# revollllt/FP8_quantization

Measured on AMD Instinct MI355X. Metric: ImageNet val images/sec, ResNet-18 FP8 approx_v9, higher is better.
Workload: dtype fp32; 1 GPU; resnet18 E4M3 approx_v9 forward (dnsmp_factor=3, withComp=False, with_s2nn2s_opt, quant_btw_mult_accu, res_quantizer, fixed ranges), ImageNet-shaped synthetic batch, random-init weights with BN statistics estimated on 4 synthetic batches; global_batch=1024, per_gpu_batch=1024, approx_macs_per_image=1814073344, parallelism=dp1

## Files before the change

### fp8_quantization_amd/csrc/fp8approx.hip

```cpp
#include <hip/hip_runtime.h>
#include <stdint.h>
#include <string.h>

#include <algorithm>
#include <atomic>
#include <cmath>
#include <cstdlib>
#include <cstdio>
#include <map>
#include <mutex>
#include <string>
#include <vector>

#include "../../include/fp8approx.h"
#include "fp8approx_common.h"
#include "fp8approx_launch.h"
#include "gemm_f8mx.h"
#include "gemm_v5mx.h"
#include "gemm_tt.h"
#include "gemm_tt16.h"
#include "gemm_dense.h"
#include "conv_tbx.h"
#include "gemm_check.h"
#include "fq_mse.h"
// ... 439 lines not shown
        const float *s = ap_sm + t * ps;
        float acc = 0.0f;
        for (int r = 0; r < kh; ++r)
            for (int c = 0; c < kw; ++c) acc += s[r * W + c];
        y[P0 + t] = acc / (float)(kh * kw);
    }
}

__global__ __launch_bounds__(256) void max_pool2d_s2k3_kernel(const float *x, float *y, int64_t planes, int H, int W,
                                                             int Ho) {
    const int Wq = W / 8;
    const int64_t total = planes * Ho * Wq;
    for (int64_t idx = (int64_t)blockIdx.x * blockDim.x + threadIdx.x; idx < total;
         idx += (int64_t)gridDim.x * blockDim.x) {
        const int q = (int)(idx % Wq);
        const int64_t t = idx / Wq;
        const int ho = (int)(t % Ho);
        const int64_t pl = t / Ho;
        const float *xp = x + pl * H * W;
        float m[4] = {-INFINITY, -INFINITY, -INFINITY, -INFINITY};
        const int c0 = 8 * q;
#pragma unroll
        for (int ky = 0; ky < 3; ++ky) {
            const int hi = 2 * ho - 1 + ky;
            if ((unsigned)hi >= (unsigned)H) continue;
            const float *r = xp + (int64_t)hi * W + c0;
            const float4 a = *reinterpret_cast<const float4 *>(r), b = *reinterpret_cast<const float4 *>(r + 4);
            const float v[9] = {c0 > 0 ? r[-1] : -INFINITY, a.x, a.y, a.z, a.w, b.x, b.y, b.z, b.w};
#pragma unroll
            for (int o = 0; o < 4; ++o)
#pragma unroll
                for (int kx = 0; kx < 3; ++kx) {
                    if (o == 0 && kx == 0 && c0 == 0) continue;
                    const float u = v[2 * o + kx];
                    m[o] = (u > m[o] || u != u) ? u : m[o];
                }
        }
        *reinterpret_cast<float4 *>(y + (pl * Ho + ho) * (int64_t)(W / 2) + 4 * q) = make_float4(m[0], m[1], m[2], m[3]);
    }
}

static void launch_f8mx(const GemmArgs &a, hipStream_t s) {
    if (a.Mw == 2) {
        launch_f8mx_xf1(a, s);
        launch_f8mx_xf2(a, s);
    } else {
        launch_f8mx_xf0(a, s);
    }
}

static int g_opt_xm_ncg = getenv("FP8A_XM_NCG") ? atoi(getenv("FP8A_XM_NCG")) : 0;
static int g_opt_xm_sign_rows = getenv("FP8A_XM_SIGN_ROWS") ? atoi(getenv("FP8A_XM_SIGN_ROWS")) : 1;
static int g_opt_xm_pipe = getenv("FP8A_XM_PIPE") ? atoi(getenv("FP8A_XM_PIPE")) != 0 : 1;
static int g_opt_fq_fast = getenv("FP8A_FQ_FAST") ? atoi(getenv("FP8A_FQ_FAST")) != 0 : 1;
static int xm_ncg(int64_t N) {
    const int forced = g_opt_xm_ncg;
    if (forced == 1 || forced == 2 || forced == 4) return forced;
    int best = 4;
    int64_t bp = (N + 63) / 64 * 64;
    for (int c : {2, 1}) {
        const int64_t pad = (N + 16 * c - 1) / (16 * c) * (16 * c);
        if (pad < bp) {
            bp = pad;
            best = c;
        }
    }
    return best;
}

static void launch_fast(int mode, const GemmArgs &a, hipStream_t s) {
    const int64_t tiles = ((a.M + BM - 1) / BM) * ((a.N + BN - 1) / BN);
    const dim3 grid((unsigned)(tiles * a.splits));
    if (mode == TM_V5) {
        if (a.aw && a.wfmt == 4) launch_v5mx(a, s);
        else launch_fast_p0(TM_V5, false, a, grid, s);
        return;
    }
    if (mode == TM_QAMAA) {
        launch_fast_p0(TM_QAMAA, false, a, grid, s);
        return;
    }
    if (a.aw && (a.wfmt == 1 || a.wfmt == 2)) {
        launch_tt(a, grid, s);
        return;
    }
    if (mode == TM_F8) {
        if (a.aw || a.af32) launch_f8mx(a, s);
        else launch_fast_p3(TM_F8, false, a, grid, s);
        return;
    }
    const bool s2n = a.flags & F_S2N, q = a.flags & F_QBMA, gc = a.flags & F_GCLIP;
    if (s2n) q ? launch_fast_p3(mode, gc, a, grid, s) : launch_fast_p2(mode, gc, a, grid, s);
    else q ? launch_fast_p1(mode, gc, a, grid, s) : launch_fast_p0(mode, gc, a, grid, s);
}

static int check_format(int E, int Mw) {
    if (E < 1 || Mw < 1 || Mw > 5 || E > 6 || E + Mw > 8)
        return fail(FP8A_EFORMAT, "Invalid combination of expo_width and mant_width");
    return FP8A_OK;
}

constexpr size_t FLAG_BYTES = 256;

enum { PATH_F8MX = 0, PATH_TT = 1, PATH_TT16 = 2, PATH_FAST = 3, PATH_EXACT = 4, PATH_DENSE = 5, PATH_V5MX = 6,
       PATH_N = 7 };
static std::atomic<uint64_t> g_paths[PATH_N];
// ... 311 lines not shown
        ++g_paths[PATH_EXACT];
        gemm_exact_kernel<<<eblocks, 256, 0, s>>>(a);
        return hip_check("fp8a exact gemm launch");
    }
    if (ws == nullptr || ws_bytes < FLAG_BYTES) return fail(FP8A_EINVAL, "matmul workspace too small");
    static const bool no_units = getenv("FP8A_NO_UNITS") != nullptr;
    const size_t head = ws_bytes >= head_bytes(a.M, a.N) ? head_bytes(a.M, a.N) : FLAG_BYTES;
    ArenaLease lease;
    const int cap = stream_capturing(s);
    if (cap < 0) return hip_check("fp8a stream capture query");
    if (cap ? !capture_lease(s, ws, ws_bytes, head, lease) : !flag_arena(s, head_bytes(a.M, a.N), lease))
        return lease_error();
    a.flag = lease.mine;
    a.flag_out = (uint32_t *)ws;
    a.arena_clr = lease.clr;
    a.arena_clr16 = lease.clr16;
    a.nur = (a.M + 63) / 64;
    a.nuc = (a.N + 63) / 64;
    a.urow = no_units || (cap && head < head_bytes(a.M, a.N)) ? nullptr : (uint8_t *)a.flag + FLAG_BYTES;
    a.ucol = no_units ? nullptr : a.urow + a.nur;
    a.utile = no_units ? nullptr : a.ucol + a.nuc;
    a.splits = choose_splits(a.M, a.N, a.K);
    if (a.splits > 1 && ws_bytes < head + splitk_bytes(a.M, a.N, a.K)) a.splits = 1;
    const int64_t kt = (a.K + BK - 1) / BK;
    a.kchunk = ((kt + a.splits - 1) / a.splits) * BK;
    a.part = a.splits > 1 ? (float *)((char *)ws + head) : nullptr;
    a.aw = nullptr;
    const bool tt = mode != TM_F8 && tt_form(a.Mw, a.flags, a.tab);
    const bool v5mx = v5mx_form(a.Mw, a.flags, mode);
    if ((mode == TM_F8 || tt || v5mx) && !no_mx()) {
        const int64_t kpad = kt * BK, npad = (a.N + BN - 1) / BN * BN;
        const size_t off = head + (a.splits > 1 ? splitk_bytes(a.M, a.N, a.K) : 0);
        const int64_t a_words = xm_a_words(a);
        const WordImage wi = word_image(a.H, a.W, a.ph, a.pw);
        a.awH = wi.H; a.awW = wi.W; a.awph = wi.ph; a.awpw = wi.pw;
        const bool fits32 = a_words < (1ll << 30) && kpad * npad * 4 < (1ll << 32);
        if (fits32 && ws_bytes >= off + xm_operand_bytes(a.N, a.K, a_words)) {
            char *base = (char *)ws + off;
            a.aw = (const uint32_t *)base;
            a.awld = kpad;
            a.bqw = (const uint2 *)(base + align256((size_t)a_words * 4));
            a.lutw = (const uint32_t *)(base + align256((size_t)a_words * 4) + xm_b_bytes(kpad, npad));
            a.ebr = (const uint16_t *)((const char *)a.lutw + 16384);
            a.xm_vmin = 0;
            if (mode == TM_F8) (void)xm_table_form(a.tab, a.Mw, &a.xm_vmin);
            a.npad = npad;
            a.ttf7 = 0;
            for (int i = 0; tt && i < (1 << (2 * a.Mw)); ++i) a.ttf7 |= a.tab.raw[i] < 0;
            a.wfmt = v5mx ? 4 : tt ? (tt16_form(a.Mw, a.ttf7, a.K) ? 2 : 1) : 0;
            if (a.wfmt == 1 && !g_opt_tt_band) a.ebr = nullptr;
            a.xncg = tt ? 4 : xm_ncg(a.N);
            a.xm_signs = g_opt_xm_sign_rows;
            a.xm_pipe = g_opt_xm_pipe;
            a.skcnt = nullptr;
            if (a.splits > 1 && g_opt_splitk_fixup && a.wfmt == 0 && a.Mw == 3) {
                a.skcnt = (uint32_t *)((char *)ws + head + splitk_part_bytes(a.splits, a.M, a.N));
                a.sk_words = splitk_counter_words(a.M, a.N);
            }
            const bool use_img = a.in_img != nullptr && !tt && a.conv && a.fqin.mx != nullptr;
            if (use_img) a.aw = a.in_img + 64;
            a.af32 = !tt && !v5mx && !use_img && xm_af32(a) ? 1 : 0;
            const int64_t rows = a.conv ? a.M / (a.Ho * a.Wo) : a.M, cols = a_words / std::max<int64_t>(rows, 1);
            dim3 ga((unsigned)std::min<int64_t>((cols + 255) / 256, 64), (unsigned)std::min<int64_t>(rows, 1024));
            {
                const int64_t hw = a.H * a.W, lim0 = a.conv ? cols : a.K, istride = a.conv ? a.Cin * hw : a.lda;
                const float *in0 = a.conv ? a.X + a.cbase * hw : a.A;
                const bool flat = !(a.conv && (a.awph | a.awpw)) && lim0 % 4 == 0 && cols % 4 == 0 && istride % 4 == 0 &&
                                  ((uintptr_t)in0 & 15) == 0 && ((uintptr_t)a.aw & 15) == 0;
                if (flat) ga = dim3((unsigned)std::max<int64_t>(1, std::min<int64_t>((a_words / 4 + 1023) / 1024, 8192)), 1);
            }
            if (use_img) {
                a.gate = a.in_img;
                xm_decode_a<<<ga.y == 1 ? dim3(std::min(ga.x, 512u)) : dim3(std::min(ga.x, 8u), std::min(ga.y, 64u)), 256, 0,
                              s>>>(a);
                a.gate = nullptr;
            } else if (!a.af32) {
                xm_decode_a<<<ga, 256, 0, s>>>(a);
            }
            if (v5mx) {
                const unsigned gb = (unsigned)std::min<int64_t>((kpad * npad + 255) / 256, 4096);
                v5mx_decode_b<<<gb, 256, 0, s>>>(a, kpad);
            } else if (tt) {
                const unsigned gb = (unsigned)std::min<int64_t>((kpad * npad + 255) / 256, 4096);
                tt_decode_b<<<gb, 256, 0, s>>>(a, kpad);
            } else {
                const unsigned gb = (unsigned)std::min<int64_t>((kpad * npad / 2 + 255) / 256, 4096);
                xm_decode_b<<<gb, 256, 0, s>>>(a, kpad);
            }
            rc = hip_check("fp8a operand pre-decode launch");
            if (rc) return rc;
        }
    }
    if (a.fqin.mx && !a.aw)
        return fail(FP8A_EINVAL, "internal: fused input quantization without the matrix-core path");
    if (mode == TM_F8 && a.Mw != 3 && !a.aw) mode = mode0;
    ++g_paths[!a.aw ? PATH_FAST : a.wfmt == 0 ? PATH_F8MX : a.wfmt == 1 ? PATH_TT : a.wfmt == 4 ? PATH_V5MX : PATH_TT16];
    if (a.em.w != nullptr && (a.em.form == 2 || (a.aw && a.wfmt != 0 && a.splits == 1) || a.post_act == 2)) {
        if (dev_fill(a.em.invalid, 1, sizeof(uint32_t), s) != hipSuccess) return hip_check("fp8a word image header");
        a.em.w = nullptr;
    }
    KernelEv kev{};
    if (g_ktime && !cap) {
        kev.a = pool_event();
        kev.b = pool_event();
        kev.path = !a.aw ? PATH_FAST : a.wfmt == 0 ? PATH_F8MX : a.wfmt == 1 ? PATH_TT : a.wfmt == 4 ? PATH_V5MX : PATH_TT16;
        kev.dispatches = (a.aw && ((a.wfmt == 0 && a.Mw == 2) || a.wfmt == 2)) ? 2 : 1;
// ... 264 lines not shown
size_t fp8a_flag_arena_slot_bytes(fp8a_stream_t stream) {
    int dev = 0;
    if (hipGetDevice(&dev) != hipSuccess) return 0;
    std::lock_guard<std::mutex> lock(g_arena_mu);
    const auto it = g_arenas.find({dev, (uintptr_t)stream});
    return it == g_arenas.end() ? 0 : it->second.slot;
}

int fp8a_kernel_timing(int enable) {
    const int old = g_ktime ? 1 : 0;
    g_ktime = enable != 0;
    return old;
}

int fp8a_kernel_time(double *out, int reset) {
    if (out == nullptr) return fail(FP8A_EINVAL, "null pointer");
    for (int i = 0; i < 4 * PATH_N; ++i) out[i] = 0.0;
    for (const KernelEv &e : g_kev) {
        if (hipEventSynchronize(e.b) != hipSuccess) return hip_check("fp8a_kernel_time");
        float ms = 0.0f;
        if (hipEventElapsedTime(&ms, e.a, e.b) != hipSuccess) return hip_check("fp8a_kernel_time");
        out[4 * e.path] += ms;
        out[4 * e.path + 1] += 1.0;
        out[4 * e.path + 2] += e.dispatches;
        out[4 * e.path + 3] += e.macs;
    }
    if (reset) {
        for (const KernelEv &e : g_kev) {
            g_evpool.push_back(e.a);
            g_evpool.push_back(e.b);
        }
        g_kev.clear();
    }
    return FP8A_OK;
}

static int g_opt_mse_group = getenv("FP8A_MSE_GROUP") ? atoi(getenv("FP8A_MSE_GROUP")) != 0 : 1;

int fp8a_set_option(const char *name, int value) {
    if (name == nullptr) return fail(FP8A_EINVAL, "null pointer");
    if (strcmp(name, "xm_ncg") == 0) {
        const int old = g_opt_xm_ncg;
        g_opt_xm_ncg = value;
        return old;
    }
    if (strcmp(name, "xm_sign_rows") == 0) {
        const int old = g_opt_xm_sign_rows;
        g_opt_xm_sign_rows = value != 0;
        return old;
    }
    if (strcmp(name, "xm_pipe") == 0) {
        const int old = g_opt_xm_pipe;
        g_opt_xm_pipe = value != 0;
        return old;
    }
    if (strcmp(name, "splitk_fixup") == 0) {
        const int old = g_opt_splitk_fixup;
        g_opt_splitk_fixup = value != 0;
        return old;
    }
    if (strcmp(name, "splitk") == 0) {
        const int old = g_opt_splitk;
        g_opt_splitk = std::max(0, value);
        return old;
    }
    if (strcmp(name, "fq_fast") == 0) {
        const int old = g_opt_fq_fast;
        g_opt_fq_fast = value != 0;
        return old;
    }
    if (strcmp(name, "af32_maxct") == 0) {
        const int old = g_opt_af32_maxct;
        g_opt_af32_maxct = std::max(0, value);
        return old;
    }
    if (strcmp(name, "tt_band") == 0) {
        const int old = g_opt_tt_band;
        g_opt_tt_band = value;
        return old;
    }
    if (strcmp(name, "tt16_mink") == 0) {
        const int old = g_opt_tt16_mink;
        g_opt_tt16_mink = std::max(0, value);
        return old;
    }
    if (strcmp(name, "tbx_rw") == 0) {
        const int old = g_opt_tbx_rw;
        g_opt_tbx_rw = value;
        return old;
    }
    if (strcmp(name, "tbs") == 0) {
        const int old = g_opt_tbs;
        g_opt_tbs = value;
        return old;
    }
    if (strcmp(name, "dw_lds") == 0) {
        const int old = g_opt_dw_lds;
        g_opt_dw_lds = std::min(65536, std::max(4096, value));
        return old;
    }
    if (strcmp(name, "dw_target") == 0) {
        const int old = g_opt_dw_target;
        g_opt_dw_target = std::max(256, value);
        return old;
    }
    if (strcmp(name, "dn_direct") == 0) {
// ... 1316 lines not shown
```

### fp8_quantization_amd/csrc/fp8approx_common.h

```cpp
#pragma once
#include <hip/hip_runtime.h>
#include <stdint.h>
#include <string.h>

#include <algorithm>
#include <atomic>
#include <cmath>
#include <cstdlib>
#include <cstdio>
#include <string>

#include "../../include/fp8approx.h"
#include "fp8approx_device.h"

namespace fp8a {

enum TMode : int { TM_NONE = 0, TM_W1U = 1, TM_W2S1 = 2, TM_W2U1 = 3, TM_W2S2 = 4, TM_W2U2 = 5, TM_LUT = 6,
                   TM_QAMAA = 7 ,
                   TM_V5 = 8 ,
                   TM_F8 = 9  };

struct TablePack {
    uint32_t rows[64][2];
    int8_t raw[1024];
// ... 32 lines not shown
}
__device__ __forceinline__ FqFast fq_fast_k(float mx, float bias, int M) {
    return FqFast{(uint32_t)(128 - (int)bias) << 23, ((uint32_t)(23 - M) << 23) | 0x00400000u, mx};
}
__device__ __forceinline__ float fq_apply_fast(float xc, const FqFast &k) {
    const uint32_t u = __float_as_uint(xc);
    const float C = __uint_as_float(max(u & 0x7F800000u, k.emn) + k.cadd);
    const float q = (xc + C) - C;
    return __uint_as_float((__float_as_uint(q) & 0x7FFFFFFFu) | (u & 0x80000000u));
}
template <bool FQF>
__device__ __forceinline__ float fq_apply_f(float v, float mx, float bias, int M, int sign_bits, const FqFast &k) {
    if (FQF) {
        const float xc = fminf(fmaxf(v, sign_bits ? -k.mx : 0.0f), k.mx);
        return k.emn ? fq_apply_fast(xc, k) : fq_apply_lit(xc, bias, M);
    }
    return fq_apply_lit(fminf(fmaxf(v, sign_bits ? -mx : 0.0f), mx), bias, M);
}

struct EmitW {
    uint32_t *w;
    uint32_t *invalid;
    int awH, awW, awph, awpw;
    int Wo;
    uint32_t hw_mul, hw_shift, wo_mul, wo_shift;
    uint32_t hw;
    FqIn fq;
    const int32_t *bR;
    int Mw;
    int form;
};

struct GemmArgs {
    const float *A;
    int64_t lda;
    const float *B;
    int64_t sbk, sbn;
    float *C;
    int64_t ldc;
    int64_t M, N, K;
    int E, Mw;
    uint32_t kexp, kdc;
    const int32_t *bA;
    const int32_t *bB;
    int64_t bBs;
    const int32_t *bR;
    uint32_t flags;
    int nchw;
    int64_t hw, ctot, coff;
    uint32_t *flag;
    uint8_t *urow, *ucol, *utile;
    int64_t nur, nuc;
    int splits;
    int64_t kchunk;
    float *part;
    uint32_t *skcnt;
    int64_t sk_words;
    int conv;
    const float *X;
    int64_t Cin, H, W, Ho, Wo, cbase;
    int kh, kw, sh, sw, ph, pw, dh, dw;
    uint32_t kk_mul, kk_shift, kw_mul, kw_shift;
    const float *qmax;
    int qE, qM, qsign;
    const float2 *ep;
    int ep_act;
    float ep_lo, ep_hi;
    const uint32_t *aw;
    int64_t awld, aw_c;
    int64_t awH, awW;
    int awph, awpw;
    int wfmt;
    int ttf7;
    int af32;
    int xncg;
    int xm_signs;
    int fq_fast;
    const uint2 *bqw;
    const uint32_t *lutw;
    const uint16_t *ebr;
    int xm_vmin;
    int xm_pipe;
    int64_t npad;
    FqIn fqin;
    float *fq_bias;
    int32_t *fq_ibias;
    const float *res;
    int post_act;
    float post_lo, post_hi;
    FqIn post_fq;
    EmitW em;
    const uint32_t *gate;
    const uint32_t *in_img;
    TablePack tab;
    uint32_t *flag_out;
    uint4 *arena_clr;
    uint32_t arena_clr16;
    float *post_bout;
    int32_t *post_ibout;
};

constexpr uint32_t FB_ANY = 1u, FB_ALL = 32u;
constexpr uint32_t FB_HALF = 64u;
constexpr uint8_t UT_EXACT = 1u, UT_HALF = 2u;

__device__ __forceinline__ uint32_t fb_bits(const GemmArgs &p, bool all = false) {
// ... 430 lines not shown
```

### fp8_quantization_amd/csrc/gemm_f8mx.h

```cpp
#pragma once
#include "fp8approx_common.h"

namespace fp8a {

typedef int xm_v8i __attribute__((ext_vector_type(8)));
typedef float xm_v16f __attribute__((ext_vector_type(16)));
typedef float xm_v4f __attribute__((ext_vector_type(4)));
typedef short xm_s2 __attribute__((ext_vector_type(2)));
typedef unsigned short xm_u2 __attribute__((ext_vector_type(2)));
typedef __bf16 xm_b2 __attribute__((ext_vector_type(2)));

constexpr int XM_NPAIR = 81;
constexpr int XM_LUT_WORDS = XM_NPAIR * 8;
static_assert(XM_SIGN_BIT == (8u << XM_ROW_SHIFT) && XM_ROW_MASK == (15u << XM_ROW_SHIFT), "A word row field");
constexpr int XBK = 8;
constexpr int XM_TTK = 16 * 32 + 16;
constexpr int XM_CP = BN + 1;

template <int XF>
struct XmFmt {
    static constexpr int M = XF ? 2 : 3;
    static constexpr int XB = XF ? 15 : 7;
};
__device__ __forceinline__ bool xm_needs_halving(const GemmArgs &p, bool af32, int bA, int bR) {
// ... 362 lines not shown
                if ((cb & 0x7FFFFFFFu) == 0u) continue;
                const int e = (int)((cb >> 23) & 0xFFu) - 127;
                emax = max(emax, e);
                emin = min(emin, e);
            }
            const_cast<uint16_t *>(p.ebr)[i] = (uint16_t)((emax + 128) | ((emin + 128) << 8));
            bmax = max(bmax, (uint32_t)(emax + 128));
        }
        wave_max_atomic(p.flag + 2, bmax);
    }
    if (__syncthreads_or(bad ? 1 : 0) && threadIdx.x == 0) atomicOr(p.flag, fb_bits(p, biasbad));
}
#else
__global__ void xm_decode_b(const GemmArgs p, int64_t kpad);
#endif

#if FP8A_OWN_F8MX
#ifndef FP8A_CLOCK_STAMP
#define FP8A_CLOCK_STAMP 0
#endif
__device__ unsigned long long g_clk[3];
__device__ unsigned long long g_xm_sign[2];
#if FP8A_CLOCK_STAMP
#define FP8A_CLK_BEGIN const uint64_t clk_t0 = __builtin_amdgcn_s_memtime(), clk_r0 = __builtin_amdgcn_s_memrealtime();
#define FP8A_CLK_END                                                                                   \
    if (threadIdx.x == 0) {                                                                            \
        const uint64_t clk_t1 = __builtin_amdgcn_s_memtime(), clk_r1 = __builtin_amdgcn_s_memrealtime(); \
        atomicAdd(&g_clk[0], (unsigned long long)(clk_t1 - clk_t0));                                   \
        atomicAdd(&g_clk[1], (unsigned long long)(clk_r1 - clk_r0));                                   \
        atomicAdd(&g_clk[2], 1ull);                                                                    \
    }
#else
#define FP8A_CLK_BEGIN
#define FP8A_CLK_END
#endif
#ifndef XM_WAVES
#define XM_WAVES 5
#endif
#ifndef XM_WAVES_PLAIN
#define XM_WAVES_PLAIN (XM_BDMA ? 6 : XM_WAVES)
#endif
template <bool AF32, bool EMIT> struct XmWaves { static constexpr int value = XM_WAVES; };
template <> struct XmWaves<false, false> { static constexpr int value = XM_WAVES_PLAIN; };
#ifndef XM_PIPE_EMIT64
#define XM_PIPE_EMIT64 1
#endif
template <int NCG, bool EMIT, bool FIX> struct XmPipe { static constexpr int value = 1; };
#ifndef XM_PIPE_PLAIN64
#define XM_PIPE_PLAIN64 2
#endif
template <> struct XmPipe<4, false, false> { static constexpr int value = XM_PIPE_PLAIN64; };
template <> struct XmPipe<4, true, false> { static constexpr int value = XM_PIPE_EMIT64; };
template <bool EMIT> struct XmPipe<1, EMIT, true> { static constexpr int value = 0; };
template <int NCG, int RB, bool AF32, int XF, bool EMIT, bool FIX = false, int PIPE = 0>
__global__ __launch_bounds__(256, (XmWaves<AF32, EMIT>::value)) void gemm_f8mx_kernel(const GemmArgs p) {
    static_assert(PIPE == 0 || (!AF32 && XF != 2), "PIPE: the word-staged plain forms only");
    using Cf = XmCfg<NCG, RB>;
    constexpr int XM = XmFmt<XF>::M, XB = XmFmt<XF>::XB;
    constexpr int NT = Cf::NT, BMT = Cf::BMT, BNT = Cf::BNT, TTK = Cf::TTK, APR = Cf::APR;
    constexpr int BU = Cf::BU, NBU = Cf::NBU, TXN = Cf::TXN, SR = Cf::SR, CP = Cf::CP;
    __shared__ __attribute__((aligned(16))) typename Cf::Smem smu;
    auto &sm = smu.st;
    FP8A_CLK_BEGIN

    const int tid = threadIdx.x, lane = tid & 63, wv = tid >> 6;
    const int wvu = __builtin_amdgcn_readfirstlane(wv);
    const int wc = wvu % NCG, wr = wvu / NCG;
    const int64_t num_mt = (p.M + BMT - 1) / BMT;
    const int64_t tiles = num_mt * ((p.N + BNT - 1) / BNT);
    const int64_t bid = (int64_t)blockIdx.x % tiles, split = (int64_t)blockIdx.x / tiles;
    const int64_t m0 = (bid % num_mt) * BMT;
    const int64_t n0 = (bid / num_mt) * BNT;
    bool both = true;
    if (!AF32 && p.xm_signs)
        both = __any(__hip_atomic_load(p.flag + (lane < XM_SIGN_NW ? XM_SIGN_W0 + lane : 3), __ATOMIC_RELAXED,
                                       __HIP_MEMORY_SCOPE_WORKGROUP) != 0u) != 0;
    if (XF != 2 && blockIdx.x == 0 && tid == 0) atomicAdd(&g_xm_sign[both ? 1 : 0], 1ull);
    if (XF == 2 && !xm_half_gate(p, m0, BMT, n0, BNT)) return;
    const int kbeg = (int)(split * p.kchunk), kend = (int)min(p.K, (int64_t)kbeg + p.kchunk), K32 = (int)p.K;
    const int bR = *p.bR;
    float fmx = 0.0f, fbias = 0.0f;
    int bA = 0;
    bool abad = false, biasbad = false;
    if (AF32) {
        fmx = p.fqin.mx ? *p.fqin.mx : 0.0f;
        fbias = p.fqin.mx ? fq_bias(fmx, p.fqin.E, p.fqin.M) : 0.0f;
        bA = p.fqin.mx ? (int)fbias : *p.bA;
        if (p.fqin.mx && blockIdx.x == 0 && tid == 0) {
            *p.fq_bias = fbias;
            *p.fq_ibias = bA;
        }
        biasbad = !(xm_bias_ok(bA) && xm_bias_ok(bR));
    }
    const uint32_t emnA = (uint32_t)(128 - bA) << 23;

    for (int e = 4 * tid; e < XM_LUT_WORDS; e += 4 * NT)
        *reinterpret_cast<uint4 *>(&sm.lut[e]) = *reinterpret_cast<const uint4 *>(&p.lutw[e]);

    const uint32_t hq8 = (uint32_t)(p.npad / 2) * 8u;
    const int q4 = tid & 3, btx = (tid >> 3) % TXN;
    constexpr int BKU = 2 * (NT / (8 * TXN));
    const int bkk0 = 2 * (tid / (8 * TXN)) + ((tid >> 2) & 1);
    const uint32_t boff0 = (uint32_t)(kbeg + bkk0) * hq8 + (uint32_t)(n0 / 2 + 2 * btx) * 8u;
    const bool build = NBU % NT == 0 || tid < NBU;
#if XM_BDMA
    const float *bsrc = reinterpret_cast<const float *>(p.bqw) +
                        ((size_t)(kbeg + tid / TXN) * (hq8 / 4) + (size_t)(n0 / 2 + 2 * (tid % TXN)) * 2);
    (void)boff0;
#else
// ... 125 lines not shown
        for (int i = 0; i < APR; ++i)
            *reinterpret_cast<uint2 *>(&sm.aw[akp][2 * (arow + 64 * i)]) = make_uint2(wa[i][0], wa[i][1]);
        if (build) {
            auto pk = [](uint32_t v, xm_u2 ad) { return __builtin_bit_cast(uint32_t, __builtin_bit_cast(xm_u2, v) + ad); };
            auto unit_b = [&](int u) {
#if XM_BDMA
                return sm.bw[(bkk0 + u * BKU) * TXN + btx];
#else
                return wbq[u];
#endif
            };
            if (both) {
#pragma unroll
                for (int u = 0; u < BU; ++u) {
                    const uint4 b = unit_b(u);
                    const uint2 s0 = *reinterpret_cast<const uint2 *>(lut + b.y + 8 * q4);
                    const uint2 s1 = *reinterpret_cast<const uint2 *>(lut + b.w + 8 * q4);
                    const xm_u2 a0 = __builtin_bit_cast(xm_u2, b.x), a1 = __builtin_bit_cast(xm_u2, b.z);
                    const xm_u2 n0 = __builtin_bit_cast(xm_u2, b.x ^ 0x80008000u), n1 = __builtin_bit_cast(xm_u2, b.z ^ 0x80008000u);
                    uint32_t *d = &sm.tt[bkk0 + u * BKU][btx * 32 + q4 * 4];
                    *reinterpret_cast<uint4 *>(d) = make_uint4(pk(s0.x, a0), pk(s1.x, a1), pk(s0.y, a0), pk(s1.y, a1));
                    *reinterpret_cast<uint4 *>(d + 16) = make_uint4(pk(s0.x, n0), pk(s1.x, n1), pk(s0.y, n0), pk(s1.y, n1));
                }
            } else {
#pragma unroll
                for (int u = 0; u < BU; ++u) {
                    uint4 b = unit_b(u);
                    asm volatile("" : "+v"(b.x), "+v"(b.z));
                    const uint2 s0 = *reinterpret_cast<const uint2 *>(lut + b.y + 8 * q4);
                    const uint2 s1 = *reinterpret_cast<const uint2 *>(lut + b.w + 8 * q4);
                    const xm_u2 a0 = __builtin_bit_cast(xm_u2, b.x), a1 = __builtin_bit_cast(xm_u2, b.z);
                    uint32_t *d = &sm.tt[bkk0 + u * BKU][btx * 32 + q4 * 4];
                    *reinterpret_cast<uint4 *>(d) = make_uint4(pk(s0.x, a0), pk(s1.x, a1), pk(s0.y, a0), pk(s1.y, a1));
                }
            }
        }
        __syncthreads();
        if (k0 + XBK < kend) load_tile(k0 + XBK);

        {
            const int r16 = lane & 15, g = lane >> 4;
            const uint32_t base = wvo + (uint32_t)(2 * g) * (uint32_t)(TTK * 4);
            const char *tt0 = reinterpret_cast<const char *>(&sm.tt[0][0]);
            uint32_t thr = 0u;
            if (XF == 2) {
                const int64_t ng = p.npad / 16, e0 = (int64_t)(k0 + 2 * g) * ng + (n0 / 16 + wc);
                const uint32_t r0 = p.ebr[e0], r1 = p.ebr[e0 + ng];
                const uint32_t thi0 = (uint32_t)max(112 + (int)(r0 & 0xFFu) - 128, 0);
                const uint32_t thi1 = (uint32_t)max(112 + (int)(r1 & 0xFFu) - 128, 0);
                const uint32_t tok0 = (uint32_t)min(max(140 + (int)(r0 >> 8) - 128 + p.xm_vmin, 0), 252);
                const uint32_t tok1 = (uint32_t)min(max(140 + (int)(r1 >> 8) - 128 + p.xm_vmin, 0), 252);
                thr = thi0 | (thi1 << 8) | (tok0 << 16) | (tok1 << 24);
            }
            if constexpr (PIPE != 0) {
                auto tread = [&](uint32_t aword, int h, uint2(&v)[4]) {
                    uint32_t a;
                    asm("v_and_or_b32 %0, %1, %2, %3" : "=v"(a) : "v"(aword), "s"(XM_ROW_MASK), "v"(base));
                    __builtin_assume((a & 7u) == 0u);
                    xm_lds_u64 *ttk = (xm_lds_u64 *)(tt0 + h * TTK * 4);
#pragma unroll
                    for (int c = 0; c < 4; ++c) {
                        const uint64_t w = ttk[(a >> 3) + 16 * c];
                        v[c] = make_uint2((uint32_t)w, (uint32_t)(w >> 32));
                    }
                };
                auto conv = [&](const uint2(&v)[4], uint32_t aword, int h) {
                    const float sc = __uint_as_float(aword);
#pragma unroll
                    for (int c = 0; c < 4; ++c) {
                        xm_s2 cv;
                        if (XF) {
                            asm("v_cvt_scalef32_pk_bf8_bf16 %0, %1, %2" : "=v"(cv) : "v"(v[c].x), "v"(sc));
                            cv = __builtin_amdgcn_cvt_scalef32_pk_bf8_bf16(cv, __builtin_bit_cast(xm_b2, v[c].y), sc, true);
                        } else {
                            asm("v_cvt_scalef32_pk_fp8_bf16 %0, %1, %2" : "=v"(cv) : "v"(v[c].x), "v"(sc));
                            cv = __builtin_amdgcn_cvt_scalef32_pk_fp8_bf16(cv, __builtin_bit_cast(xm_b2, v[c].y), sc, true);
                        }
                        av[4 * h + c] = __builtin_bit_cast(int, cv);
                    }
                };
                auto aread = [&](int b) {
                    const uint64_t w = *(xm_lds_u64 *)&sm.aw[g][2 * (16 * (RB * wr + b) + r16)];
                    return make_uint2((uint32_t)w, (uint32_t)(w >> 32));
                };
                uint2 va[4], vb[4];
                uint2 awc = aread(0), awn = awc;
                if (PIPE == 2) tread(awc.x, 0, va);
#pragma unroll
                for (int b = 0; b < RB; ++b) {
                    if (b + 1 < RB) awn = aread(b + 1);
                    if (PIPE == 2) {
                        tread(awc.y, 1, vb);
                        __builtin_amdgcn_sched_barrier(0);
                        conv(va, awc.x, 0);
                        __builtin_amdgcn_sched_barrier(0);
                        if (b + 1 < RB) tread(awn.x, 0, va);
                        __builtin_amdgcn_sched_barrier(0);
                        conv(vb, awc.y, 1);
                    } else {
                        __builtin_amdgcn_sched_barrier(0);
                        tread(awc.x, 0, va);
                        conv(va, awc.x, 0);
                        tread(awc.y, 1, va);
                        conv(va, awc.y, 1);
                    }
                    dq[b] = __builtin_amdgcn_mfma_scale_f32_16x16x128_f8f6f4(av, sel, dq[b], XF ? 1 : 0, 0, 0, 127, 0, 127);
                    __builtin_amdgcn_sched_barrier(0);
// ... 32 lines not shown
                        const uint64_t w = ttk[(a >> 3) + 16 * c];
                        v[c] = make_uint2((uint32_t)w, (uint32_t)(w >> 32));
                    }
                    const float sc = __uint_as_float(awh[h]);
#pragma unroll
                    for (int c = 0; c < 4; ++c) {
                        xm_s2 cv;
                        if (XF) {
                            asm("v_cvt_scalef32_pk_bf8_bf16 %0, %1, %2" : "=v"(cv) : "v"(v[c].x), "v"(sc));
                            cv = __builtin_amdgcn_cvt_scalef32_pk_bf8_bf16(cv, __builtin_bit_cast(xm_b2, v[c].y), sc, true);
                        } else {
                            asm("v_cvt_scalef32_pk_fp8_bf16 %0, %1, %2" : "=v"(cv) : "v"(v[c].x), "v"(sc));
                            cv = __builtin_amdgcn_cvt_scalef32_pk_fp8_bf16(cv, __builtin_bit_cast(xm_b2, v[c].y), sc, true);
                        }
                        av[4 * h + c] = __builtin_bit_cast(int, cv);
                    }
                }
                dq[b] = __builtin_amdgcn_mfma_scale_f32_16x16x128_f8f6f4(av, sel, dq[b], XF ? 1 : 0, 0, 0, sca, 0, 127);
            }
        }
#if XM_BDMA
        __builtin_amdgcn_s_waitcnt(0x0F70);
#endif
        __syncthreads();
    }

    bool nan = false;
#pragma unroll
    for (int b = 0; b < RB; ++b)
#pragma unroll
        for (int i = 0; i < 4; ++i) nan |= !__builtin_isfinite(dq[b][i]);
    const bool tnan = __syncthreads_or(nan ? 1 : 0) != 0;
    const bool tbad = AF32 && __syncthreads_or((abad || biasbad) ? 1 : 0) != 0;
    if ((tnan || tbad) && tid == 0) {
        if (XF == 1 && tnan && xm_needs_halving(p, AF32, AF32 ? bA : 0, bR)) {
            fb_tile(p, m0, BMT, n0, UT_HALF);
            atomicOr(p.flag, FB_HALF);
            if (tbad) atomicOr(p.flag, fb_bits(p, biasbad));
        } else {
            if (tnan) fb_tile(p, m0, BMT, n0, XF == 2 ? (uint8_t)(UT_EXACT | UT_HALF) : UT_EXACT);
            atomicOr(p.flag, fb_bits(p, biasbad));
        }
    }

    const float f8S = __uint_as_float((uint32_t)min(max(127 + XB - bR, 1), 254) << 23);
    float *ct = smu.ct;
    const StoreCtx sc = p.splits == 1 ? store_ctx<EMIT>(p) : StoreCtx{};
    const int ety = tid & 15, etx = tid >> 4, cb = etx % (BNT / 4), sub = etx / (BNT / 4);
#pragma unroll
    for (int h = 0; h < BMT / SR; ++h) {
        if (h > 0) __syncthreads();
#pragma unroll
        for (int b = 0; b < RB; ++b) {
            const int rb = 16 * (RB * wr + b) - SR * h;
            if (rb >= 0 && rb < SR) {
#pragma unroll
                for (int i = 0; i < 4; ++i)
                    ct[(rb + 4 * (lane >> 4) + i) * CP + 16 * wc + (lane & 15)] = dq[b][i] * f8S;
            }
        }
        __syncthreads();
        float acc[TM][TN];
#pragma unroll
        for (int i = 0; i < TM; ++i)
#pragma unroll
            for (int j = 0; j < TN; ++j) acc[i][j] = ct[(64 * sub + ety * TM + i) * CP + cb * TN + j];
        store_tile<EMIT, !EMIT, true>(p, split, m0 + SR * h + 64 * sub, n0, ety, cb, acc, sc);
    }
    if (FIX && p.skcnt != nullptr) {
        asm volatile("s_waitcnt vmcnt(0)" ::: "memory");
        __syncthreads();
        if (tid == 0) {
            __builtin_amdgcn_fence(__ATOMIC_RELEASE, "agent");
            asm volatile("s_waitcnt vmcnt(0)" ::: "memory");
            const uint32_t t = __hip_atomic_fetch_add(p.skcnt + bid, 1u, __ATOMIC_RELAXED, __HIP_MEMORY_SCOPE_AGENT);
            const bool mine = t == (uint32_t)p.splits - 1u;
            if (mine) {
                __builtin_amdgcn_fence(__ATOMIC_ACQUIRE, "agent");
                asm volatile("s_waitcnt vmcnt(0)" ::: "memory");
            }
            ct[0] = mine ? 1.0f : 0.0f;
        }
        __syncthreads();
        if (ct[0] != 0.0f) splitk_finish_tile<EMIT, !EMIT, BMT, BNT, NT>(p, m0, n0, tid);
    }
    FP8A_CLK_END
}
#endif

}
```

### fp8_quantization_amd/csrc/k_f8mx.hip

```cpp
#ifndef FP8A_XF_PART
#error "k_f8mx.hip is compiled once per part: -DFP8A_XF_PART=0..2"
#endif
#define FP8A_OWN_F8MX 1
#define FP8A_OWN_F8MX_DECODE (FP8A_XF_PART == 0)
#include "fp8approx_launch.h"
#include "gemm_f8mx.h"

namespace fp8a {

template <int NCG, int RB, int XF>
static void launch_shape(const GemmArgs &a, hipStream_t s) {
    using Cf = XmCfg<NCG, RB>;
    const int64_t xt = ((a.M + Cf::BMT - 1) / Cf::BMT) * ((a.N + Cf::BNT - 1) / Cf::BNT);
    const dim3 g((unsigned)(xt * a.splits));
    const bool emit = a.em.w != nullptr && (a.splits == 1 || a.skcnt != nullptr);
    if constexpr (XF != 2) {
        if (a.xm_pipe && !a.af32) {
            if constexpr (XF == 0) {
                if (a.skcnt != nullptr) {
                    if (emit) gemm_f8mx_kernel<NCG, RB, false, XF, true, true, XmPipe<NCG, true, true>::value><<<g, Cf::NT, 0, s>>>(a);
                    else gemm_f8mx_kernel<NCG, RB, false, XF, false, true, XmPipe<NCG, false, true>::value><<<g, Cf::NT, 0, s>>>(a);
                    return;
                }
            }
            if (emit) gemm_f8mx_kernel<NCG, RB, false, XF, true, false, XmPipe<NCG, true, false>::value><<<g, Cf::NT, 0, s>>>(a);
            else gemm_f8mx_kernel<NCG, RB, false, XF, false, false, XmPipe<NCG, false, false>::value><<<g, Cf::NT, 0, s>>>(a);
            return;
        }
    }
    if constexpr (XF == 0) {
        if (a.skcnt != nullptr) {
            if (a.af32) {
                if (emit) gemm_f8mx_kernel<NCG, RB, true, XF, true, true><<<g, Cf::NT, 0, s>>>(a);
                else gemm_f8mx_kernel<NCG, RB, true, XF, false, true><<<g, Cf::NT, 0, s>>>(a);
            } else {
                if (emit) gemm_f8mx_kernel<NCG, RB, false, XF, true, true><<<g, Cf::NT, 0, s>>>(a);
                else gemm_f8mx_kernel<NCG, RB, false, XF, false, true><<<g, Cf::NT, 0, s>>>(a);
            }
            return;
        }
    }
    if (a.af32) {
        if (emit) gemm_f8mx_kernel<NCG, RB, true, XF, true><<<g, Cf::NT, 0, s>>>(a);
        else gemm_f8mx_kernel<NCG, RB, true, XF, false><<<g, Cf::NT, 0, s>>>(a);
    } else {
        if (emit) gemm_f8mx_kernel<NCG, RB, false, XF, true><<<g, Cf::NT, 0, s>>>(a);
        else gemm_f8mx_kernel<NCG, RB, false, XF, false><<<g, Cf::NT, 0, s>>>(a);
    }
}

template <int XF>
static void launch_xf(const GemmArgs &a, hipStream_t s) {
    if (a.xncg == 1) {
        launch_shape<1, 4, XF>(a, s);
    } else if constexpr (XF == 2) {
        launch_shape<2, 4, XF>(a, s);
    } else {
        if (a.xncg == 2) launch_shape<2, 4, XF>(a, s);
        else launch_shape<4, 8, XF>(a, s);
    }
}

static int clock_read(unsigned long long *v, bool reset) {
    if (hipMemcpyFromSymbol(v, HIP_SYMBOL(g_clk), 3 * sizeof(unsigned long long)) != hipSuccess) return -1;
    if (reset) {
        const unsigned long long z[3] = {0, 0, 0};
        if (hipMemcpyToSymbol(HIP_SYMBOL(g_clk), z, sizeof(z)) != hipSuccess) return -1;
    }
    return 0;
}

static int signs_read(unsigned long long *v, bool reset) {
    if (hipMemcpyFromSymbol(v, HIP_SYMBOL(g_xm_sign), 2 * sizeof(unsigned long long)) != hipSuccess) return -1;
    if (reset) {
// ... 22 lines not shown
```

Baseline: 13610 images/s.

## Assign each wave two full row blocks across all column groups in f8mx PIPE kernel

Adds a WROWS variant of the 128x64 pipelined f8mx GEMM. In it each wave owns two 16-row blocks and iterates over all four column groups, instead of owning a fixed column group across eight row blocks. A-operand LDS words are read once per row block and reused across the column groups, while the table reads change to per-column-group indexing. The epilogue mapping is adjusted to match. The variant is on by default through a new env option and raises register and scheduling complexity.

```diff
diff --git a/fp8_quantization_amd/csrc/fp8approx.hip b/fp8_quantization_amd/csrc/fp8approx.hip
--- a/fp8_quantization_amd/csrc/fp8approx.hip
+++ b/fp8_quantization_amd/csrc/fp8approx.hip
@@ -515,6 +515,7 @@
 static int g_opt_xm_ncg = getenv("FP8A_XM_NCG") ? atoi(getenv("FP8A_XM_NCG")) : 0;
 static int g_opt_xm_sign_rows = getenv("FP8A_XM_SIGN_ROWS") ? atoi(getenv("FP8A_XM_SIGN_ROWS")) : 1;
 static int g_opt_xm_pipe = getenv("FP8A_XM_PIPE") ? atoi(getenv("FP8A_XM_PIPE")) != 0 : 1;
+static int g_opt_xm_wave_rows = getenv("FP8A_XM_WAVE_ROWS") ? atoi(getenv("FP8A_XM_WAVE_ROWS")) != 0 : 1;
 static int g_opt_fq_fast = getenv("FP8A_FQ_FAST") ? atoi(getenv("FP8A_FQ_FAST")) != 0 : 1;
 static int xm_ncg(int64_t N) {
     const int forced = g_opt_xm_ncg;
@@ -932,6 +933,7 @@
             a.xncg = tt ? 4 : xm_ncg(a.N);
             a.xm_signs = g_opt_xm_sign_rows;
             a.xm_pipe = g_opt_xm_pipe;
+            a.xm_wave_rows = g_opt_xm_wave_rows;
             a.skcnt = nullptr;
             if (a.splits > 1 && g_opt_splitk_fixup && a.wfmt == 0 && a.Mw == 3) {
                 a.skcnt = (uint32_t *)((char *)ws + head + splitk_part_bytes(a.splits, a.M, a.N));
@@ -1302,6 +1304,11 @@
     if (strcmp(name, "xm_pipe") == 0) {
         const int old = g_opt_xm_pipe;
         g_opt_xm_pipe = value != 0;
+        return old;
+    }
+    if (strcmp(name, "xm_wave_rows") == 0) {
+        const int old = g_opt_xm_wave_rows;
+        g_opt_xm_wave_rows = value != 0;
         return old;
     }
     if (strcmp(name, "splitk_fixup") == 0) {
diff --git a/fp8_quantization_amd/csrc/fp8approx_common.h b/fp8_quantization_amd/csrc/fp8approx_common.h
--- a/fp8_quantization_amd/csrc/fp8approx_common.h
+++ b/fp8_quantization_amd/csrc/fp8approx_common.h
@@ -108,6 +108,7 @@
     uint8_t *urow, *ucol, *utile;
     int64_t nur, nuc;
     int splits;
+    int xm_wave_rows;
     int64_t kchunk;
     float *part;
     uint32_t *skcnt;
diff --git a/fp8_quantization_amd/csrc/gemm_f8mx.h b/fp8_quantization_amd/csrc/gemm_f8mx.h
--- a/fp8_quantization_amd/csrc/gemm_f8mx.h
+++ b/fp8_quantization_amd/csrc/gemm_f8mx.h
@@ -438,9 +438,10 @@
 template <> struct XmPipe<4, false, false> { static constexpr int value = XM_PIPE_PLAIN64; };
 template <> struct XmPipe<4, true, false> { static constexpr int value = XM_PIPE_EMIT64; };
 template <bool EMIT> struct XmPipe<1, EMIT, true> { static constexpr int value = 0; };
-template <int NCG, int RB, bool AF32, int XF, bool EMIT, bool FIX = false, int PIPE = 0>
+template <int NCG, int RB, bool AF32, int XF, bool EMIT, bool FIX = false, int PIPE = 0, bool WROWS = false>
 __global__ __launch_bounds__(256, (XmWaves<AF32, EMIT>::value)) void gemm_f8mx_kernel(const GemmArgs p) {
     static_assert(PIPE == 0 || (!AF32 && XF != 2), "PIPE: the word-staged plain forms only");
+    static_assert(!WROWS || (NCG == 4 && RB == 8 && PIPE != 0 && !FIX), "WROWS: the 128 x 64 PIPE instances");
     using Cf = XmCfg<NCG, RB>;
     constexpr int XM = XmFmt<XF>::M, XB = XmFmt<XF>::XB;
     constexpr int NT = Cf::NT, BMT = Cf::BMT, BNT = Cf::BNT, TTK = Cf::TTK, APR = Cf::APR;
@@ -672,7 +673,85 @@
                 const uint32_t tok1 = (uint32_t)min(max(140 + (int)(r1 >> 8) - 128 + p.xm_vmin, 0), 252);
                 thr = thi0 | (thi1 << 8) | (tok0 << 16) | (tok1 << 24);
             }
-            if constexpr (PIPE != 0) {
+            if constexpr (WROWS) {
+                const uint32_t rbase = (uint32_t)(2 * g) * (uint32_t)(TTK * 4);
+                auto addr = [&](uint32_t aword) {
+                    uint32_t a;
+                    asm("v_and_or_b32 %0, %1, %2, %3" : "=v"(a) : "v"(aword), "s"(XM_ROW_MASK), "v"(rbase));
+                    return a;
+                };
+                auto tread = [&](uint32_t a, int cg, int h, uint2(&v)[4]) {
+                    __builtin_assume((a & 7u) == 0u);
+                    xm_lds_u64 *ttk = (xm_lds_u64 *)(tt0 + h * TTK * 4 + cg * 512);
+#pragma unroll
+                    for (int c = 0; c < 4; ++c) {
+                        const uint64_t w = ttk[(a >> 3) + 16 * c];
+                        v[c] = make_uint2((uint32_t)w, (uint32_t)(w >> 32));
+                    }
+                };
+                auto conv = [&](const uint2(&v)[4], uint32_t aword, int h) {
+                    const float sc = __uint_as_float(aword);
+#pragma unroll
+                    for (int c = 0; c < 4; ++c) {
+                        xm_s2 cv;
+                        if (XF) {
+                            asm("v_cvt_scalef32_pk_bf8_bf16 %0, %1, %2" : "=v"(cv) : "v"(v[c].x), "v"(sc));
+                            cv = __builtin_amdgcn_cvt_scalef32_pk_bf8_bf16(cv, __builtin_bit_cast(xm_b2, v[c].y), sc, true);
+                        } else {
+                            asm("v_cvt_scalef32_pk_fp8_bf16 %0, %1, %2" : "=v"(cv) : "v"(v[c].x), "v"(sc));
+                            cv = __builtin_amdgcn_cvt_scalef32_pk_fp8_bf16(cv, __builtin_bit_cast(xm_b2, v[c].y), sc, true);
+                        }
+                        av[4 * h + c] = __builtin_bit_cast(int, cv);
+                    }
+                };
+                auto aread = [&](int rb) {
+                    const uint64_t w = *(xm_lds_u64 *)&sm.aw[g][2 * (16 * (2 * wvu + rb) + r16)];
+                    return make_uint2((uint32_t)w, (uint32_t)(w >> 32));
+                };
+                uint2 va[4], vb[4];
+                uint2 awc = aread(0), awn = awc;
+                uint32_t a0 = addr(awc.x), a1 = addr(awc.y);
+                if (PIPE == 2) tread(a0, 0, 0, va);
+#pragma unroll
+                for (int rb = 0; rb < 2; ++rb) {
+                    uint32_t a0n = a0, a1n = a1;
+#pragma unroll
+                    for (int cg = 0; cg < 4; ++cg) {
+                        if (PIPE == 2) {
+                            tread(a1, cg, 1, vb);
+                            if (cg == 3 && rb + 1 < 2) awn = aread(rb + 1);
+                            __builtin_amdgcn_sched_barrier(0);
+                            conv(va, awc.x, 0);
+                            __builtin_amdgcn_sched_barrier(0);
+                            if (cg + 1 < 4) {
+                                tread(a0, cg + 1, 0, va);
+                            } else if (rb + 1 < 2) {
+                                a0n = addr(awn.x);
+                                a1n = addr(awn.y);
+                                tread(a0n, 0, 0, va);
+                            }
+                            __builtin_amdgcn_sched_barrier(0);
+                            conv(vb, awc.y, 1);
+                        } else {
+                            __builtin_amdgcn_sched_barrier(0);
+                            tread(a0, cg, 0, va);
+                            conv(va, awc.x, 0);
+                            tread(a1, cg, 1, va);
+                            if (cg == 3 && rb + 1 < 2) awn = aread(rb + 1);
+                            conv(va, awc.y, 1);
+                        }
+                        dq[4 * rb + cg] = __builtin_amdgcn_mfma_scale_f32_16x16x128_f8f6f4(av, sel, dq[4 * rb + cg], XF ? 1 : 0, 0, 0, 127, 0, 127);
+                        __builtin_amdgcn_sched_barrier(0);
+                    }
+                    awc = awn;
+                    if (PIPE == 1 && rb + 1 < 2) {
+                        a0n = addr(awc.x);
+                        a1n = addr(awc.y);
+                    }
+                    a0 = a0n;
+                    a1 = a1n;
+                }
+            } else if constexpr (PIPE != 0) {
                 auto tread = [&](uint32_t aword, int h, uint2(&v)[4]) {
                     uint32_t a;
                     asm("v_and_or_b32 %0, %1, %2, %3" : "=v"(a) : "v"(aword), "s"(XM_ROW_MASK), "v"(base));
@@ -811,11 +890,12 @@
         if (h > 0) __syncthreads();
 #pragma unroll
         for (int b = 0; b < RB; ++b) {
-            const int rb = 16 * (RB * wr + b) - SR * h;
+            const int rb = 16 * (WROWS ? 2 * wvu + b / 4 : RB * wr + b) - SR * h;
+            const int cg = WROWS ? b % 4 : wc;
             if (rb >= 0 && rb < SR) {
 #pragma unroll
                 for (int i = 0; i < 4; ++i)
-                    ct[(rb + 4 * (lane >> 4) + i) * CP + 16 * wc + (lane & 15)] = dq[b][i] * f8S;
+                    ct[(rb + 4 * (lane >> 4) + i) * CP + 16 * cg + (lane & 15)] = dq[b][i] * f8S;
             }
         }
         __syncthreads();
diff --git a/fp8_quantization_amd/csrc/k_f8mx.hip b/fp8_quantization_amd/csrc/k_f8mx.hip
--- a/fp8_quantization_amd/csrc/k_f8mx.hip
+++ b/fp8_quantization_amd/csrc/k_f8mx.hip
@@ -20,6 +20,13 @@
                 if (a.skcnt != nullptr) {
                     if (emit) gemm_f8mx_kernel<NCG, RB, false, XF, true, true, XmPipe<NCG, true, true>::value><<<g, Cf::NT, 0, s>>>(a);
                     else gemm_f8mx_kernel<NCG, RB, false, XF, false, true, XmPipe<NCG, false, true>::value><<<g, Cf::NT, 0, s>>>(a);
+                    return;
+                }
+            }
+            if constexpr (NCG == 4) {
+                if (a.xm_wave_rows) {
+                    if (emit) gemm_f8mx_kernel<NCG, RB, false, XF, true, false, XmPipe<NCG, true, false>::value, true><<<g, Cf::NT, 0, s>>>(a);
+                    else gemm_f8mx_kernel<NCG, RB, false, XF, false, false, XmPipe<NCG, false, false>::value, true><<<g, Cf::NT, 0, s>>>(a);
                     return;
                 }
             }
```

New measurement: 14050 images/s, median of 6. +3.2%, better.
